# CogitoNTNU/geoguessr-ai

Hardware: AMD Instinct MI355X
Metric: images/sec TinyViT-21M-224 train, 4-heading batch (higher is better)
Workload: dtype fp32 (bf16x3 split MFMA); 1 GPU; tiny_vit_21m_224 4x224x224 panoramas, fwd+bwd+AdamW, soft-CE over 12647 geocells, freeze_all_but_last_stage, DropPath, train-mode BN; panoramas_per_gpu=256, images_per_gpu=1024, global_batch_panoramas=256, parallelism=dp1, precision=fp32_split

## Files before the change

geoguessr-ai_amd/csrc/gemm_split3.hip:

```cpp
#include "common.h"
#include <type_traits>
#include <algorithm>
#include <stdlib.h>
#include <string.h>
#include "../../include/gg.h"
#include "../../include/gg_wgrad_resident.h"
#include "../../include/gg_conv_dgrad_parity.h"

namespace {

struct Split3Params {
    const bf16* A; int64_t lda, plane_a;
    const float* Af; int64_t ldaf;
    const bf16* B; int64_t ldb, plane_b;
    float* C; int64_t ldc;
    const float* bias;
    int M, N, K, tilesM, tilesN;
    int act; float* preact;
    const float* rowscale; int rows_per_scale;
    const float* residual; int64_t ldr;
    const float* dact_preact; int dact;
    bf16* c_planes; int64_t ldp;
    const float* a_stat; const float* a_gamma; const float* a_beta; int a_act;
    float* colstats;
// ... 901 lines not shown
#pragma unroll
        for (int it = 0; it < 4; ++it) r[it] = load1(it, 1);
#pragma unroll
        for (int i = 0; i < 6; ++i) {
            bf16x4 p1, p2, p3;
            split2(t0[i], 0, p1, p2, p3); split2(t0[i], 2, p1, p2, p3);
            store3(i < 4 ? i : i + 3, Yim, p1, p2, p3);
        }
    }
    union Fr { s3_s4 h[2]; bf16x8 v; };
    Fr yf[3][3], xf[2][3];
    auto rd_y = [&](const bf16* ycur, int pl, int t) {
#pragma unroll
        for (int half = 0; half < 2; ++half)
            yf[pl][t].h[half] = __builtin_amdgcn_ds_read_tr16_b64_v4i16((__attribute__((address_space(3))) s3_s4*)(ycur + pl * PY + yoff[t] + half * 512));
    };
    auto rd_x = [&](int ring, int j) {
#pragma unroll
        for (int pl = 0; pl < 3; ++pl)
#pragma unroll
            for (int half = 0; half < 2; ++half)
                xf[ring][pl].h[half] = __builtin_amdgcn_ds_read_tr16_b64_v4i16((__attribute__((address_space(3))) s3_s4*)(Xim + pl * PX + xoff[j] + half * 512));
    };
    auto phase = [&](auto j0_, auto nj_, auto it0_, auto nit_, int s, bf16* ynxt) {
        constexpr int J0 = decltype(j0_)::value, NJ = decltype(nj_)::value, IT0 = decltype(it0_)::value, NIT = decltype(nit_)::value;
        constexpr int Q = 6 * NJ, S = 3 * NIT;
        constexpr int PA[6] = {0, 1, 2, 0, 1, 0}, PB[6] = {2, 1, 0, 1, 0, 0};
        bf16x4 p1, p2, p3;
#pragma unroll
        for (int jj = 0; jj < NJ; ++jj) {
            if (jj + 1 < NJ) rd_x((jj + 1) & 1, J0 + jj + 1);
#pragma unroll
            for (int g = 0; g < 6; ++g) {
#pragma unroll
                for (int nt = 0; nt < 3; ++nt)
                    acc[nt][J0 + jj] = __builtin_amdgcn_mfma_f32_16x16x32_bf16(xf[jj & 1][PA[g]].v, yf[PB[g]][nt].v, acc[nt][J0 + jj], 0, 0, 0);
                const int qi = jj * 6 + g;
                if ((qi * S) % Q < S) {
                    const int ms = (qi * S) / Q, it = IT0 + ms / 3, part = ms % 3;
                    if (part < 2) split2(r[it], 2 * part, p1, p2, p3);
                    else {
                        store3(it, ynxt, p1, p2, p3);
                        r[it] = load1(it, it >= 4 && it < 7 ? s + 1 : s + 2);
                    }
                }
                __builtin_amdgcn_sched_barrier(0);
            }
        }
    };
    for (int s = 0; s < nk; ++s) {
        const bf16* const ycur = Yim + (s & 1) * 3 * PY;
        bf16* const ynxt = Yim + ((s + 1) & 1) * 3 * PY;
        asm volatile("s_waitcnt lgkmcnt(0)" ::: "memory");
        __builtin_amdgcn_s_barrier();
        rd_x(0, 0);
#pragma unroll
        for (int t = 0; t < 3; ++t) rd_y(ycur, 2, t);
#pragma unroll
        for (int t = 0; t < 3; ++t) rd_y(ycur, 1, t);
#pragma unroll
        for (int t = 0; t < 3; ++t) rd_y(ycur, 0, t);
        phase(std::integral_constant<int, 0>{}, std::integral_constant<int, 4>{}, std::integral_constant<int, 4>{}, std::integral_constant<int, 5>{}, s, ynxt);
        asm volatile("s_waitcnt lgkmcnt(0)" ::: "memory");
        __builtin_amdgcn_s_barrier();
        rd_x(0, 4);
        phase(std::integral_constant<int, 4>{}, std::integral_constant<int, 3>{}, std::integral_constant<int, 0>{}, std::integral_constant<int, 4>{}, s, ynxt);
    }
    wait_vm<0>();
    float* out = p.part + (int64_t)slab * p.N * p.K;
#pragma unroll
    for (int nt = 0; nt < 3; ++nt) {
        const int n = 48 * wn + 16 * nt + lr;
#pragma unroll
        for (int j = 0; j < 7; ++j) {
            const int k = 16 * (wk + 4 * j) + 4 * lg;
            if (n < p.N && k < p.K) *reinterpret_cast<f32x4*>(out + (int64_t)n * p.K + k) = acc[nt][j];
        }
    }
}

struct PeDgradParams {
    const float* dy; const bf16* Bp; const float* y; const float* stat; const float* gamma; const float* beta; int act;
    float* dz; float* part;
    int H, W, Cout, tiles_per_img, total_tiles, tiles_per_block;
};
constexpr int PED_N = 48, PED_BM = 128;
__device__ __host__ __forceinline__ int ped_taps_before(int cls) { return cls == 0 ? 0 : cls == 1 ? 1 : cls == 2 ? 3 : 5; }
__global__ __launch_bounds__(256) void pe_dgrad_pack_kernel(const float* __restrict__ Wt, int64_t ldw, int Cout, bf16* __restrict__ out) {
    const int c4n = Cout / 4, total = PED_N * 9 * c4n;
    for (int i = blockIdx.x * blockDim.x + threadIdx.x; i < total; i += gridDim.x * blockDim.x) {
        const int co = (i % c4n) * 4, u = (i / c4n) % 9, c = i / (9 * c4n);
        const int cls = u < 1 ? 0 : u < 3 ? 1 : u < 5 ? 2 : 3, t = u - ped_taps_before(cls);
        const int py = cls >> 1, px = cls & 1, nx = 1 + px, ty = t / nx, tx = t % nx;
        const int ky = py ? (ty ? 0 : 2) : 1, kx = px ? (tx ? 0 : 2) : 1;
        const int Kc = Cout * (1 + py) * (1 + px);
        const f32x4 v = *reinterpret_cast<const f32x4*>(Wt + (int64_t)((ky * 3 + kx) * PED_N + c) * ldw + co);
        bf16x4 p1, p2, p3;
#pragma unroll
        for (int j = 0; j < 4; ++j) {
            bf16 s1_, s2_, s3_;
            gg_split3_rne(v[j], s1_, s2_, s3_);
            p1[j] = s1_; p2[j] = s2_; p3[j] = s3_;
        }
        bf16* q = out + (int64_t)3 * PED_N * Cout * ped_taps_before(cls) + (int64_t)c * Kc + t * Cout + co;
        *reinterpret_cast<bf16x4*>(q) = p1; *reinterpret_cast<bf16x4*>(q + PED_N * Kc) = p2; *reinterpret_cast<bf16x4*>(q + 2 * PED_N * Kc) = p3;
    }
}
__global__ __launch_bounds__(256) void pe_dgrad_split3_kernel(PeDgradParams p) {
    constexpr int BM = PED_BM, BN = PED_N, TM = 2, TN = 3, LDT = BN + 4;
    constexpr int TA = BM * S3_SK, TB = BN * S3_SK;
    constexpr int CPR = BN / 4, RPP = 256 / CPR, NR = (BM + RPP - 1) / RPP;
    extern __shared__ __attribute__((aligned(16))) bf16 s3mem[];
    bf16* const Abuf = s3mem;
    bf16* const Bbuf = s3mem + 3 * TA;
    float* const Ct = reinterpret_cast<float*>(s3mem);
    const int lane = threadIdx.x & 63, wave = __builtin_amdgcn_readfirstlane(threadIdx.x >> 6);
    const int lr = lane & 15, lg = lane >> 4;
    const int H0 = p.H >> 1, W0 = p.W >> 1, npc = H0 * W0, spt = p.Cout >> 5;
    const int dchunk = (lane & 3) ^ s3_swz(lane >> 4);
    const int kq = threadIdx.x & 7, arow = threadIdx.x >> 3;
    int ldsA[4];
#pragma unroll
    for (int j = 0; j < 4; ++j) {
        const int row = arow + 32 * j;
        ldsA[j] = row * S3_SK + (((kq >> 1) ^ s3_swz((row >> 2) & 3)) << 3) + ((kq & 1) << 2);
    }
    const int fslot = (lg ^ s3_swz((lr >> 2) & 3)) * 8;
    const int a_off = (wave * 32 + lr) * S3_SK + fslot, b_off = lr * S3_SK + fslot;
    const int chunk = threadIdx.x % CPR, r0 = threadIdx.x / CPR, c0 = chunk * 4;
    const bool elive = r0 < RPP;
    const f32x4 mu = *reinterpret_cast<const f32x4*>(p.stat + c0), rstd = *reinterpret_cast<const f32x4*>(p.stat + BN + c0);
    const f32x4 ga = *reinterpret_cast<const f32x4*>(p.gamma + c0), be = *reinterpret_cast<const f32x4*>(p.beta + c0);
    f32x4 ssum = {0.f, 0.f, 0.f, 0.f}, qsum = ssum;
    auto split2 = [&](const f32x4& v, int e0, bf16x4& p1, bf16x4& p2, bf16x4& p3) {
#pragma unroll
        for (int e = e0; e < e0 + 2; ++e) {
            bf16 s1_, s2_, s3_;
            gg_split3_rne(v[e], s1_, s2_, s3_);
            p1[e] = s1_; p2[e] = s2_; p3[e] = s3_;
        }
    };
    const int lid = gg_xcd_remap(blockIdx.x, gridDim.x);
    const int t_begin = lid * p.tiles_per_block, t_end = min(t_begin + p.tiles_per_block, p.total_tiles);
    for (int tile = t_begin; tile < t_end; ++tile) {
        const int img = tile / (4 * p.tiles_per_img), rem = tile - img * 4 * p.tiles_per_img;
        const int tin = rem >> 2, cls = rem & 3, py = cls >> 1, px = cls & 1, nx = 1 + px;
        const int Kc = p.Cout * (1 + py) * nx, nk = spt * (1 + py) * nx;
        const int q0 = tin * BM;
        const __amdgpu_buffer_rsrc_t rsA = __builtin_amdgcn_make_buffer_rsrc((void*)(p.dy + (int64_t)img * npc * p.Cout), 0, (int)((unsigned)npc * (unsigned)p.Cout * 4u), 0x00020000);
        unsigned voffA[4];
        bool yin[4], xin[4];
#pragma unroll
        for (int j = 0; j < 4; ++j) {
            const int q = q0 + arow + 32 * j, m = q / W0, n = q - m * W0;
            voffA[j] = q < npc ? (unsigned)q * (unsigned)p.Cout * 4u + kq * 16u : 0xFFFFFFF0u;
            yin[j] = m + 1 < H0; xin[j] = n + 1 < W0;
        }
        __amdgpu_buffer_rsrc_t rsB[3];
#pragma unroll
        for (int i = 0; i < 3; ++i)
            rsB[i] = __builtin_amdgcn_make_buffer_rsrc((void*)(p.Bp + (int64_t)3 * BN * p.Cout * ped_taps_before(cls) + (int64_t)i * BN * Kc), 0, (int)((unsigned)BN * (unsigned)Kc * 2u), 0x00020000);
        const unsigned voffB = (unsigned)(wave * 16 + (lane >> 2)) * (unsigned)Kc * 2u + dchunk * 16u;
        auto issue_b = [&](int st) {
            if (wave < BN / 16 && st < nk) {
                bf16* const base = Bbuf + (st & 1) * 3 * TB;
#pragma unroll
                for (int i = 0; i < 3; ++i)
                    __builtin_amdgcn_raw_ptr_buffer_load_lds(rsB[i], (__attribute__((address_space(3))) void*)(base + i * TB + wave * 512), 16, (int)voffB, st * S3_SK * 2, 0, 0);
            }
        };
        auto load_a1 = [&](int st, int j) -> f32x4 {
            const int t = st / spt, kk = (st - t * spt) * S3_SK, ty = t / nx, tx = t - ty * nx;
            const bool dyv = py && ty, dxv = px && tx;
            const int soff = (((int)dyv * W0 + (int)dxv) * p.Cout + kk) * 4;
            const bool ok = st < nk && (!dyv || yin[j]) && (!dxv || xin[j]);
            return __builtin_bit_cast(f32x4, __builtin_amdgcn_raw_buffer_load_b128(rsA, (int)(ok ? voffA[j] : 0xFFFFFFF0u), soff, 0));
        };
        auto load_a = [&](int st, f32x4 (&r)[4]) {
#pragma unroll
            for (int j = 0; j < 4; ++j) r[j] = load_a1(st, j);
        };
        f32x4 acc[TN][TM], accs[TN][TM];
#pragma unroll
        for (int i = 0; i < TN; ++i)
#pragma unroll
            for (int j = 0; j < TM; ++j) acc[i][j] = accs[i][j] = (f32x4){0.f, 0.f, 0.f, 0.f};
        f32x4 ra[2][4];
        issue_b(0);
        load_a(0, ra[0]);
        load_a(1, ra[1]);
        wait_vm<4>();
        {
            bf16x4 p1, p2, p3;
#pragma unroll
            for (int j = 0; j < 4; ++j) {
                split2(ra[0][j], 0, p1, p2, p3); split2(ra[0][j], 2, p1, p2, p3);
                *reinterpret_cast<bf16x4*>(Abuf + ldsA[j]) = p1; *reinterpret_cast<bf16x4*>(Abuf + TA + ldsA[j]) = p2; *reinterpret_cast<bf16x4*>(Abuf + 2 * TA + ldsA[j]) = p3;
            }
        }
        load_a(2, ra[0]);
        auto stage = [&](int s, f32x4 (&rnext)[4]) {
            const bf16* const curB = Bbuf + (s & 1) * 3 * TB;
            wait_vm<4>();
            asm volatile("s_waitcnt lgkmcnt(0)" ::: "memory");
            __builtin_amdgcn_s_barrier();
            issue_b(s + 1);
            bf16x8 xf[3][TM], wf[3][TN];
#pragma unroll
            for (int pl = 0; pl < 3; ++pl)
#pragma unroll
                for (int mt = 0; mt < TM; ++mt) xf[pl][mt] = *reinterpret_cast<const bf16x8*>(Abuf + pl * TA + a_off + mt * 16 * S3_SK);
            auto rd_b1 = [&](int pl, int nt) { wf[pl][nt] = *reinterpret_cast<const bf16x8*>(curB + pl * TB + b_off + nt * 16 * S3_SK); };
#pragma unroll
            for (int t = 0; t < TN; ++t) rd_b1(2, t);
            asm volatile("s_waitcnt lgkmcnt(0)" ::: "memory");
            __builtin_amdgcn_s_barrier();
            bf16x4 p1, p2, p3;
            constexpr int PA[6] = {0, 1, 2, 0, 1, 0}, PB[6] = {2, 1, 0, 1, 0, 0};
#pragma unroll
            for (int g = 0; g < 6; ++g) {
#pragma unroll
                for (int nt = 0; nt < TN; ++nt) {
#pragma unroll
                    for (int mt = 0; mt < TM; ++mt) {
                        if (g < 5) accs[nt][mt] = __builtin_amdgcn_mfma_f32_16x16x32_bf16(wf[PB[g]][nt], xf[PA[g]][mt], accs[nt][mt], 0, 0, 0);
                        else acc[nt][mt] = __builtin_amdgcn_mfma_f32_16x16x32_bf16(wf[PB[g]][nt], xf[PA[g]][mt], acc[nt][mt], 0, 0, 0);
                    }
                    constexpr int Q = 6 * TN;
                    const int qi = g * TN + nt;
                    if (g < 2 && 2 * nt < TN) { rd_b1(1 - g, 2 * nt); if (2 * nt + 1 < TN) rd_b1(1 - g, 2 * nt + 1); }
                    if ((qi * 12) % Q < 12) {
                        const int ms = (qi * 12) / Q, jj = ms / 3, part = ms % 3;
                        if (part < 2) split2(rnext[jj], 2 * part, p1, p2, p3);
                        else {
                            *reinterpret_cast<bf16x4*>(Abuf + ldsA[jj]) = p1;
                            *reinterpret_cast<bf16x4*>(Abuf + TA + ldsA[jj]) = p2;
                            *reinterpret_cast<bf16x4*>(Abuf + 2 * TA + ldsA[jj]) = p3;
                            rnext[jj] = load_a1(s + 3, jj);
                        }
                    }
                    __builtin_amdgcn_sched_barrier(0);
                }
            }
        };
        for (int s = 0; s < nk; s += 2) {
            stage(s, ra[1]);
            if (s + 1 < nk) stage(s + 1, ra[0]);
        }
        wait_vm<0>();
        f32x4 yv[NR];
        int64_t pix[NR];
#pragma unroll
        for (int i = 0; i < NR; ++i) {
            const int rr = r0 + i * RPP, q = q0 + rr;
            const bool on = elive && rr < BM && q < npc;
            const int m = on ? q / W0 : 0, n = on ? q - m * W0 : 0;
            pix[i] = on ? ((int64_t)img * p.H + 2 * m + py) * p.W + 2 * n + px : -1;
            yv[i] = on ? *reinterpret_cast<const f32x4*>(p.y + pix[i] * BN + c0) : (f32x4){0.f, 0.f, 0.f, 0.f};
        }
        asm volatile("s_waitcnt lgkmcnt(0)" ::: "memory");
        __builtin_amdgcn_s_barrier();
#pragma unroll
        for (int nt = 0; nt < TN; ++nt)
#pragma unroll
            for (int mt = 0; mt < TM; ++mt)
                *reinterpret_cast<f32x4*>(Ct + (wave * 32 + mt * 16 + lr) * LDT + nt * 16 + lg * 4) = acc[nt][mt] + accs[nt][mt];
        __syncthreads();
#pragma unroll
        for (int i = 0; i < NR; ++i) {
            if (pix[i] < 0) continue;
            const f32x4 a = *reinterpret_cast<const f32x4*>(Ct + (r0 + i * RPP) * LDT + c0);
            const f32x4 xh = (yv[i] - mu) * rstd;
            f32x4 o;
#pragma unroll
            for (int j = 0; j < 4; ++j) o[j] = a[j] * gg_act_grad_f32(fmaf(ga[j], xh[j], be[j]), p.act);
            ssum += o;
            qsum += o * xh;
            __builtin_nontemporal_store(o, reinterpret_cast<f32x4*>(p.dz + pix[i] * BN + c0));
        }
        __syncthreads();
    }
    if (elive) {
        *reinterpret_cast<f32x4*>(Ct + (r0 * 2 + 0) * BN + c0) = ssum;
        *reinterpret_cast<f32x4*>(Ct + (r0 * 2 + 1) * BN + c0) = qsum;
    }
    __syncthreads();
    if (threadIdx.x < 2 * BN) {
        float t = 0.f;
        for (int k = 0; k < RPP; ++k) t += Ct[k * 2 * BN + threadIdx.x];
        p.part[(int64_t)blockIdx.x * 2 * BN + threadIdx.x] = t;
    }
}

__global__ __launch_bounds__(256) void split3_kernel(const float* __restrict__ x, int64_t rows, int cols, int64_t ldx, bf16* __restrict__ out) {
    const int64_t n4 = rows * (cols / 4);
    const int64_t plane = rows * cols;
    for (int64_t i = blockIdx.x * (int64_t)blockDim.x + threadIdx.x; i < n4; i += (int64_t)gridDim.x * blockDim.x) {
        const int64_t r = i / (cols / 4);
        const int c = (int)(i - r * (cols / 4)) * 4;
        const f32x4 v = *reinterpret_cast<const f32x4*>(x + r * ldx + c);
        bf16x4 p1, p2, p3;
#pragma unroll
        for (int j = 0; j < 4; ++j) {
            bf16 s1_, s2_, s3_;
            gg_split3_rne(v[j], s1_, s2_, s3_);
            p1[j] = s1_; p2[j] = s2_; p3[j] = s3_;
        }
        *reinterpret_cast<bf16x4*>(out + r * cols + c) = p1;
        *reinterpret_cast<bf16x4*>(out + plane + r * cols + c) = p2;
        *reinterpret_cast<bf16x4*>(out + 2 * plane + r * cols + c) = p3;
    }
}

}

extern "C" int gg_split3_bf16(const float* x, int64_t rows, int cols, int64_t ldx, void* planes, void* stream) {
    GG_CHECK(x && planes && rows > 0 && cols > 0 && (cols & 3) == 0 && (ldx & 3) == 0 && ldx >= cols && ((uintptr_t)x & 15) == 0 && ((uintptr_t)planes & 7) == 0,
             "gg_split3_bf16: bad args (cols %% 4, ldx %% 4, 16-byte aligned x)");
    GG_PROF(GG_CAT_MOVE, 0, 10.0 * rows * cols, stream);
    const int64_t n4 = rows * (cols / 4);
    hipLaunchKernelGGL(split3_kernel, dim3((unsigned)std::min<int64_t>(gg_cdiv(n4, 256), 16384)), dim3(256), 0, (hipStream_t)stream, x, rows, cols, ldx, (bf16*)planes);
    GG_LAUNCH_CHECK();
    return 0;
}

static GgSplit3Route split3_planes_route(int M, int N) {
    const bool big = M > 128;
    GgSplit3Route r;
    r.kernel = big ? GG_SPLIT3_ROUTE_PLANES_256 : GG_SPLIT3_ROUTE_PLANES_128;
    r.tile_n = S3_BN; r.epilogue = 0; r.mapped = 0;
    r.tilesM = (int)gg_cdiv(M, big ? 256 : 128); r.tilesN = (int)gg_cdiv(N, S3_BN);
    r.lds_bytes = big ? (int64_t)2 * 3 * (256 + 128) * S3_SK * sizeof(bf16) : (int64_t)3 * S3_STAGE * sizeof(bf16);
    return r;
}
static int split3_launch(Split3Params& p, void* stream) {
    const int M = p.M, N = p.N, K = p.K;
    const GgSplit3Route r = split3_planes_route(M, N);
    void (*kern)(Split3Params) = r.kernel == GG_SPLIT3_ROUTE_PLANES_256 ? gemm_nt_split3_kernel<256, 128, 4, 2, 2> : gemm_nt_split3_kernel<128, 128, 2, 4, 3>;
    p.tilesM = r.tilesM; p.tilesN = r.tilesN;
    const size_t lds = (size_t)r.lds_bytes;
    GG_TRY(gg_allow_lds_160k(reinterpret_cast<const void*>(kern)));
    const double mn = (double)M * N;
    GG_PROF(GG_CAT_GEMM | GG_CAT_SPLIT_FLAG, 2.0 * M * (double)N * K,
            6.0 * ((double)M * K + (double)N * K) + 4.0 * mn * ((p.C != nullptr) + (p.preact != nullptr) + (p.residual != nullptr) + (p.dact_preact != nullptr)) +
                (p.c_planes ? 6.0 * mn : 0.0), stream);
    hipLaunchKernelGGL(kern, dim3((unsigned)(p.tilesM * p.tilesN)), dim3(512), lds, (hipStream_t)stream, p);
    GG_LAUNCH_CHECK();
    return 0;
}

static int split3_planes_check(const GgSplit3Args* a) {
    GG_CHECK(a && a->a_planes && a->b_planes && (a->C || a->c_planes) && a->M > 0 && a->N > 0 && a->K > 0, "gg_gemm_nt_split3: null pointer / bad shape");
    GG_CHECK((a->K & 7) == 0 && (a->lda & 7) == 0 && (a->ldb & 7) == 0 && a->lda >= a->K && a->ldb >= a->K, "gg_gemm_nt_split3: K, lda, ldb must be multiples of 8, ld >= K");
    GG_CHECK(((uintptr_t)a->a_planes & 15) == 0 && ((uintptr_t)a->b_planes & 15) == 0 && ((uintptr_t)a->C & 15) == 0 && ((uintptr_t)a->c_planes & 7) == 0,
             "gg_gemm_nt_split3: alignment");
    GG_CHECK((int64_t)256 * a->lda * 2 < ((int64_t)1 << 31) && (int64_t)256 * a->ldb * 2 < ((int64_t)1 << 31), "gg_gemm_nt_split3: row pitch too large");
    GG_CHECK((!a->C || a->ldc >= a->N) && (!a->c_planes || a->ldp >= a->N) && (!a->residual || a->ldr >= a->N), "gg_gemm_nt_split3: leading dimension too small");
    GG_CHECK((!a->preact && !a->dact_preact) || a->ldc >= a->N, "gg_gemm_nt_split3: preact / dact_preact use ldc");
    GG_CHECK(!a->rowscale || a->rows_per_scale > 0, "gg_gemm_nt_split3: rowscale needs rows_per_scale");
    GG_CHECK(!(a->dact_preact && a->act), "gg_gemm_nt_split3: act and dact_preact are exclusive");
    GG_CHECK(!a->groups_dev && !a->a_map && !a->c_map, "gg_gemm_nt_split3: row compaction is a form of gg_gemm_nt_split3_af32 only");
    return 0;
}
extern "C" int gg_gemm_nt_split3_ex(const GgSplit3Args* a, void* stream) {
    GG_TRY(split3_planes_check(a));
    Split3Params p;
    p.a_stat = p.a_gamma = p.a_beta = nullptr; p.a_act = 0;
    p.A = (const bf16*)a->a_planes; p.lda = a->lda; p.plane_a = (int64_t)a->M * a->lda; p.Af = nullptr; p.ldaf = 0;
    p.B = (const bf16*)a->b_planes; p.ldb = a->ldb; p.plane_b = (int64_t)a->N * a->ldb;
    p.C = a->C; p.ldc = a->ldc ? a->ldc : a->N; p.bias = a->bias; p.M = a->M; p.N = a->N; p.K = a->K;
    p.act = a->act; p.preact = a->preact; p.rowscale = a->rowscale; p.rows_per_scale = a->rows_per_scale; p.residual = a->residual; p.ldr = a->ldr;
    p.dact_preact = a->dact_preact; p.dact = a->dact; p.c_planes = (bf16*)a->c_planes; p.ldp = a->ldp; p.colstats = nullptr;
// ... 143 lines not shown
    GG_TRY(split3_af32_check(a, (const float*)a->a_planes, a->lda, with_colstats != 0, pro != 0));
    return split3_af32_route(a, with_colstats != 0, pro != 0, *out);
}

extern "C" int gg_gemm_tn_f32_splits(int M, int N, int K);
extern "C" int gg_gemm_tn_split3_splits(int M, int N, int K) {
    const int64_t tiles = gg_cdiv(N, 256) * gg_cdiv(K, 128);
    const int64_t cap = std::max<int64_t>(1, ((int64_t)128 << 20) / ((int64_t)N * K * 4));
    const int64_t smax = std::max<int64_t>(1, std::min<int64_t>(cap, gg_cdiv(M, 1024)));
    int64_t s = 1;
    double best = 0.0;
    for (int64_t c = 1; c <= smax && c * tiles <= 4 * 256; ++c) {
        const double eff = (double)(c * tiles) / (256.0 * (double)gg_cdiv(c * tiles, 256));
        if (eff > best + 0.02) { best = eff; s = c; }
    }
    s = std::min<int64_t>(cap, std::max<int64_t>(s, (5 * (int64_t)gg_gemm_tn_f32_splits(M, N, K) + 3) / 4));
    const int64_t rows = gg_cdiv(gg_cdiv(M, s), 32) * 32;
    return (int)gg_cdiv(M, rows);
}
extern "C" int gg_gemm_tn_split3(const float* dY, int64_t ldy, const float* X, int64_t ldx, int M, int N, int K, const float* rowscale, int rows_per_scale, float* partials,
                                 int splits, void* stream) {
    GG_CHECK(dY && X && partials && M > 0 && N > 0 && K > 0 && splits > 0, "gg_gemm_tn_split3: bad args");
    GG_CHECK((N & 3) == 0 && (K & 3) == 0 && (ldy & 3) == 0 && (ldx & 3) == 0 && ldy >= N && ldx >= K, "gg_gemm_tn_split3: N, K, ldy, ldx must be multiples of 4, ld >= columns");
    GG_CHECK(((uintptr_t)dY & 15) == 0 && ((uintptr_t)X & 15) == 0 && ((uintptr_t)partials & 15) == 0, "gg_gemm_tn_split3: operands and partials must be 16-byte aligned");
    GG_CHECK(!rowscale || rows_per_scale > 0, "gg_gemm_tn_split3: rows_per_scale");
    Split3TnParams p;
    p.dY = dY; p.ldy = ldy; p.X = X; p.ldx = ldx; p.M = M; p.N = N; p.K = K; p.rowscale = rowscale; p.rps = rows_per_scale > 0 ? rows_per_scale : 1; p.part = partials;
    p.last_scale = (M - 1) / p.rps;
    p.rows_per_split = (int)(gg_cdiv(gg_cdiv(M, splits), 32) * 32);
    GG_CHECK((int64_t)p.rows_per_split * (splits - 1) < M, "gg_gemm_tn_split3: more splits than 32-row stages");
    GG_CHECK((int64_t)p.rows_per_split * std::max(ldy, ldx) * 4 < ((int64_t)1 << 31), "gg_gemm_tn_split3: a slab exceeds the 2 GiB descriptor range");
    p.tilesN = (int)gg_cdiv(N, 256); p.tilesK = (int)gg_cdiv(K, 128);
    GG_TRY(gg_allow_lds_160k(reinterpret_cast<const void*>(gemm_tn_split3_kernel)));
    GG_PROF(GG_CAT_GEMM | GG_CAT_SPLIT_FLAG, 2.0 * M * (double)N * K, 4.0 * ((double)M * N + (double)M * K) + 8.0 * splits * (double)N * K, stream);
    hipLaunchKernelGGL(gemm_tn_split3_kernel, dim3((unsigned)(p.tilesN * p.tilesK * splits)), dim3(512), (size_t)2 * 3 * (256 / 32 + 128 / 32) * 1024 * sizeof(bf16), (hipStream_t)stream, p);
    GG_LAUNCH_CHECK();
    return 0;
}

extern "C" int gg_gemm_tn_split3_resident_fits(int N, int K) { return N > 0 && K > 0 && N <= S3R_N && K <= S3R_K; }
extern "C" int gg_gemm_tn_split3_resident_splits(int M, int N, int K) {
    GG_CHECK(M > 0 && N > 0 && K > 0, "gg_gemm_tn_split3_resident_splits: bad shape");
    GG_CHECK(gg_gemm_tn_split3_resident_fits(N, K), "gg_gemm_tn_split3_resident: the %d x %d output does not fit one workgroup (at most %d x %d)", N, K, S3R_N, S3R_K);
    const int64_t cap = std::max<int64_t>(1, ((int64_t)128 << 20) / ((int64_t)N * K * 4));
    int64_t s = std::max<int64_t>(1, std::min<int64_t>(256, M / 256));
    s = std::max<int64_t>(s, (5 * (int64_t)gg_gemm_tn_f32_splits(M, N, K) + 3) / 4);
    s = std::min<int64_t>(std::min<int64_t>(s, cap), gg_cdiv(M, 32));
    const int64_t rows = gg_cdiv(gg_cdiv(M, s), 32) * 32;
    return (int)gg_cdiv(M, rows);
}
extern "C" int gg_gemm_tn_split3_resident(const float* dY, int64_t ldy, const float* X, int64_t ldx, int M, int N, int K, float* partials, int splits, void* stream) {
    GG_CHECK(dY && X && partials && M > 0 && N > 0 && K > 0 && splits > 0, "gg_gemm_tn_split3_resident: bad args");
    GG_CHECK(gg_gemm_tn_split3_resident_fits(N, K), "gg_gemm_tn_split3_resident: the %d x %d output does not fit one workgroup (at most %d x %d)", N, K, S3R_N, S3R_K);
    GG_CHECK((N & 3) == 0 && (K & 3) == 0 && (ldy & 3) == 0 && (ldx & 3) == 0 && ldy >= N && ldx >= K, "gg_gemm_tn_split3_resident: N, K, ldy, ldx must be multiples of 4, ld >= columns");
    GG_CHECK(((uintptr_t)dY & 15) == 0 && ((uintptr_t)X & 15) == 0 && ((uintptr_t)partials & 15) == 0, "gg_gemm_tn_split3_resident: operands and partials must be 16-byte aligned");
    Split3TnResParams p;
    p.dY = dY; p.ldy = ldy; p.X = X; p.ldx = ldx; p.M = M; p.N = N; p.K = K; p.part = partials;
    p.rows_per_split = (int)(gg_cdiv(gg_cdiv(M, splits), 32) * 32);
    GG_CHECK((int64_t)p.rows_per_split * (splits - 1) < M, "gg_gemm_tn_split3_resident: more splits than 32-row stages");
    GG_CHECK(((int64_t)p.rows_per_split + 96) * std::max(ldy, ldx) * 4 < ((int64_t)1 << 31), "gg_gemm_tn_split3_resident: a slab exceeds the 2 GiB descriptor range");
    GG_TRY(gg_allow_lds_160k(reinterpret_cast<const void*>(gemm_tn_split3_resident_kernel)));
    GG_PROF(GG_CAT_GEMM | GG_CAT_SPLIT_FLAG, 2.0 * M * (double)N * K, 4.0 * ((double)M * N + (double)M * K) + 8.0 * splits * (double)N * K, stream);
    hipLaunchKernelGGL(gemm_tn_split3_resident_kernel, dim3((unsigned)splits), dim3(512), (size_t)3 * (S3R_K / 32 + 2 * (S3R_N / 32)) * 1024 * sizeof(bf16), (hipStream_t)stream, p);
    GG_LAUNCH_CHECK();
    return 0;
}

extern "C" int gg_conv3x3s2_dgrad_fits(int H, int W, int Cin, int Cout) {
    return H > 0 && W > 0 && (H & 1) == 0 && (W & 1) == 0 && Cin == PED_N && Cout >= 32 && (Cout & 31) == 0 && (int64_t)(H / 2) * (W / 2) * Cout * 4 < ((int64_t)1 << 31);
}
extern "C" int64_t gg_conv3x3s2_dgrad_planes_bytes(int Cin, int Cout) { return (int64_t)3 * 9 * Cin * Cout * (int64_t)sizeof(bf16); }
extern "C" int gg_conv3x3s2_dgrad_bnbwd_split3(const float* dy, const float* Wt, int64_t ldw, const float* y, const float* stat, const float* gamma, const float* beta, int act,
                                               float* dz, float* part, int nparts, void* planes, int B, int H, int W, int Cin, int Cout, void* stream) {
    GG_CHECK(dy && Wt && y && stat && gamma && beta && dz && part && planes && nparts > 0 && nparts <= 65535 && B > 0, "gg_conv3x3s2_dgrad_bnbwd_split3: bad args");
    GG_CHECK(gg_conv3x3s2_dgrad_fits(H, W, Cin, Cout), "gg_conv3x3s2_dgrad_bnbwd_split3: needs an even input map, Cin = %d and Cout a multiple of 32 (got %d x %d, Cin %d, Cout %d)",
             PED_N, H, W, Cin, Cout);
    GG_CHECK(ldw >= Cout && (ldw & 3) == 0, "gg_conv3x3s2_dgrad_bnbwd_split3: ldw must be a multiple of 4, >= Cout");
    GG_CHECK(((uintptr_t)dy & 15) == 0 && ((uintptr_t)Wt & 15) == 0 && ((uintptr_t)y & 15) == 0 && ((uintptr_t)dz & 15) == 0 && ((uintptr_t)stat & 15) == 0 &&
             ((uintptr_t)gamma & 15) == 0 && ((uintptr_t)beta & 15) == 0 && ((uintptr_t)planes & 15) == 0, "gg_conv3x3s2_dgrad_bnbwd_split3: operands must be 16-byte aligned");
    PeDgradParams p;
    p.dy = dy; p.Bp = (const bf16*)planes; p.y = y; p.stat = stat; p.gamma = gamma; p.beta = beta; p.act = act; p.dz = dz; p.part = part;
    p.H = H; p.W = W; p.Cout = Cout;
    const int64_t npc = (int64_t)(H / 2) * (W / 2);
    p.tiles_per_img = (int)gg_cdiv(npc, PED_BM);
    const int64_t total = (int64_t)B * 4 * p.tiles_per_img;
    GG_CHECK(total < ((int64_t)1 << 31), "gg_conv3x3s2_dgrad_bnbwd_split3: too many tiles");
    p.total_tiles = (int)total;
    p.tiles_per_block = (int)gg_cdiv(total, nparts);
    const double M0 = (double)B * npc;
    {
        GG_PROF(GG_CAT_MOVE, 0, 4.0 * 9 * Cin * Cout + 6.0 * 9 * Cin * Cout, stream);
        hipLaunchKernelGGL(pe_dgrad_pack_kernel, dim3((unsigned)gg_cdiv((int64_t)PED_N * 9 * (Cout / 4), 256)), dim3(256), 0, (hipStream_t)stream, Wt, ldw, Cout, (bf16*)planes);
        GG_LAUNCH_CHECK();
    }
    GG_PROF(GG_CAT_GEMM | GG_CAT_SPLIT_FLAG, 2.0 * M0 * 9.0 * Cin * Cout, 4.0 * M0 * Cout + 6.0 * 9 * Cin * Cout + 2.0 * 4.0 * 4.0 * M0 * Cin + 8.0 * nparts * Cin, stream);
    hipLaunchKernelGGL(pe_dgrad_split3_kernel, dim3((unsigned)nparts), dim3(256), (size_t)(3 * PED_BM + 6 * PED_N) * S3_SK * sizeof(bf16), (hipStream_t)stream, p);
    GG_LAUNCH_CHECK();
    return 0;
}
```

Before: 5815 images/s.

## Stage a split dy spatial tile in LDS once and reuse it across all nine taps

Result: no change. 5835 images/s (median of 6 runs) (+0.3%).

```diff
diff --git a/geoguessr-ai_amd/csrc/gemm_split3.hip b/geoguessr-ai_amd/csrc/gemm_split3.hip
--- a/geoguessr-ai_amd/csrc/gemm_split3.hip
+++ b/geoguessr-ai_amd/csrc/gemm_split3.hip
@@ -1007,18 +1007,21 @@
 struct PeDgradParams {
     const float* dy; const bf16* Bp; const float* y; const float* stat; const float* gamma; const float* beta; int act;
     float* dz; float* part;
-    int H, W, Cout, tiles_per_img, total_tiles, tiles_per_block;
+    int H, W, Cout, tiles_x, tiles_per_img, total_tiles, tiles_per_block;
 };
-constexpr int PED_N = 48, PED_BM = 128;
+constexpr int PED_N = 48, PED_TW = 14, PED_FW = 16, PED_TH = 4, PED_RING = 3;
+constexpr int PED_BT = PED_N * S3_SK;
 __device__ __host__ __forceinline__ int ped_taps_before(int cls) { return cls == 0 ? 0 : cls == 1 ? 1 : cls == 2 ? 3 : 5; }
+__host__ __forceinline__ size_t ped_lds_bytes(int th, int ring, int Cout) {
+    return (size_t)4 * PED_N * sizeof(float) + ((size_t)3 * (Cout / 32) * (th + 1) * PED_FW * S3_SK + (size_t)ring * 3 * PED_BT) * sizeof(bf16);
+}
 __global__ __launch_bounds__(256) void pe_dgrad_pack_kernel(const float* __restrict__ Wt, int64_t ldw, int Cout, bf16* __restrict__ out) {
-    const int c4n = Cout / 4, total = PED_N * 9 * c4n;
+    const int c4n = Cout / 4, spt = Cout >> 5, total = PED_N * 9 * c4n;
     for (int i = blockIdx.x * blockDim.x + threadIdx.x; i < total; i += gridDim.x * blockDim.x) {
         const int co = (i % c4n) * 4, u = (i / c4n) % 9, c = i / (9 * c4n);
         const int cls = u < 1 ? 0 : u < 3 ? 1 : u < 5 ? 2 : 3, t = u - ped_taps_before(cls);
         const int py = cls >> 1, px = cls & 1, nx = 1 + px, ty = t / nx, tx = t % nx;
         const int ky = py ? (ty ? 0 : 2) : 1, kx = px ? (tx ? 0 : 2) : 1;
-        const int Kc = Cout * (1 + py) * (1 + px);
         const f32x4 v = *reinterpret_cast<const f32x4*>(Wt + (int64_t)((ky * 3 + kx) * PED_N + c) * ldw + co);
         bf16x4 p1, p2, p3;
 #pragma unroll
@@ -1027,192 +1030,182 @@
             gg_split3_rne(v[j], s1_, s2_, s3_);
             p1[j] = s1_; p2[j] = s2_; p3[j] = s3_;
         }
-        bf16* q = out + (int64_t)3 * PED_N * Cout * ped_taps_before(cls) + (int64_t)c * Kc + t * Cout + co;
-        *reinterpret_cast<bf16x4*>(q) = p1; *reinterpret_cast<bf16x4*>(q + PED_N * Kc) = p2; *reinterpret_cast<bf16x4*>(q + 2 * PED_N * Kc) = p3;
-    }
-}
+        const int ks = co >> 5, kk = co & 31;
+        bf16* q = out + ((int64_t)(u * spt + ks) * 3 * PED_N + c) * S3_SK + ((((kk >> 3) ^ s3_swz((c >> 2) & 3)) << 3) | (kk & 7));
+        *reinterpret_cast<bf16x4*>(q) = p1; *reinterpret_cast<bf16x4*>(q + PED_BT) = p2; *reinterpret_cast<bf16x4*>(q + 2 * PED_BT) = p3;
+    }
+}
+template <int TH, int R>
 __global__ __launch_bounds__(256) void pe_dgrad_split3_kernel(PeDgradParams p) {
-    constexpr int BM = PED_BM, BN = PED_N, TM = 2, TN = 3, LDT = BN + 4;
-    constexpr int TA = BM * S3_SK, TB = BN * S3_SK;
-    constexpr int CPR = BN / 4, RPP = 256 / CPR, NR = (BM + RPP - 1) / RPP;
+    constexpr int BN = PED_N, TW = PED_TW, FW = PED_FW, TM = TH / 4, TN = 3, NPIX = (TH + 1) * FW, SB = 3 * PED_BT;
+    static_assert(TH % 4 == 0 && R >= 3 && R - 1 <= 9, "one or two tile rows per wave; the ring is filled from the first tile's stages");
     extern __shared__ __attribute__((aligned(16))) bf16 s3mem[];
-    bf16* const Abuf = s3mem;
-    bf16* const Bbuf = s3mem + 3 * TA;
-    float* const Ct = reinterpret_cast<float*>(s3mem);
+    float* const bnt = reinterpret_cast<float*>(s3mem);
+    bf16* const Aimg = s3mem + 4 * BN * 2;
     const int lane = threadIdx.x & 63, wave = __builtin_amdgcn_readfirstlane(threadIdx.x >> 6);
     const int lr = lane & 15, lg = lane >> 4;
-    const int H0 = p.H >> 1, W0 = p.W >> 1, npc = H0 * W0, spt = p.Cout >> 5;
-    const int dchunk = (lane & 3) ^ s3_swz(lane >> 4);
-    const int kq = threadIdx.x & 7, arow = threadIdx.x >> 3;
-    int ldsA[4];
-#pragma unroll
-    for (int j = 0; j < 4; ++j) {
-        const int row = arow + 32 * j;
-        ldsA[j] = row * S3_SK + (((kq >> 1) ^ s3_swz((row >> 2) & 3)) << 3) + ((kq & 1) << 2);
-    }
-    const int fslot = (lg ^ s3_swz((lr >> 2) & 3)) * 8;
-    const int a_off = (wave * 32 + lr) * S3_SK + fslot, b_off = lr * S3_SK + fslot;
-    const int chunk = threadIdx.x % CPR, r0 = threadIdx.x / CPR, c0 = chunk * 4;
-    const bool elive = r0 < RPP;
-    const f32x4 mu = *reinterpret_cast<const f32x4*>(p.stat + c0), rstd = *reinterpret_cast<const f32x4*>(p.stat + BN + c0);
-    const f32x4 ga = *reinterpret_cast<const f32x4*>(p.gamma + c0), be = *reinterpret_cast<const f32x4*>(p.beta + c0);
-    f32x4 ssum = {0.f, 0.f, 0.f, 0.f}, qsum = ssum;
-    auto split2 = [&](const f32x4& v, int e0, bf16x4& p1, bf16x4& p2, bf16x4& p3) {
-#pragma unroll
-        for (int e = e0; e < e0 + 2; ++e) {
-            bf16 s1_, s2_, s3_;
-            gg_split3_rne(v[e], s1_, s2_, s3_);
-            p1[e] = s1_; p2[e] = s2_; p3[e] = s3_;
-        }
-    };
+    const int H0 = p.H >> 1, W0 = p.W >> 1, npc = H0 * W0, spt = p.Cout >> 5, nst = 9 * spt;
+    const int PS = spt * NPIX * S3_SK;
+    bf16* const Bring = Aimg + 3 * PS;
+    float* const red = reinterpret_cast<float*>(Aimg);
     const int lid = gg_xcd_remap(blockIdx.x, gridDim.x);
-    const int t_begin = lid * p.tiles_per_block, t_end = min(t_begin + p.tiles_per_block, p.total_tiles);
+    const int t_begin = min(lid * p.tiles_per_block, p.total_tiles), t_end = min(t_begin + p.tiles_per_block, p.total_tiles);
+    const int gtotal = (t_end - t_begin) * nst;
+    if (threadIdx.x < BN) {
+        bnt[threadIdx.x] = p.stat[threadIdx.x]; bnt[BN + threadIdx.x] = p.stat[BN + threadIdx.x];
+        bnt[2 * BN + threadIdx.x] = p.gamma[threadIdx.x]; bnt[3 * BN + threadIdx.x] = p.beta[threadIdx.x];
+    }
+    const __amdgpu_buffer_rsrc_t rsB = __builtin_amdgcn_make_buffer_rsrc((void*)p.Bp, 0, (int)((unsigned)nst * SB * 2u), 0x00020000);
+    const unsigned voffB = (unsigned)(wave * 512 + lane * 8) * 2u;
+    int gi = 0, bsi = 0, sloti = 0;
+    auto issue_b = [&]() {
+        if (wave < BN / 16 && gi < gtotal) {
+            bf16* const base = Bring + sloti * SB;
+#pragma unroll
+            for (int i = 0; i < 3; ++i)
+                __builtin_amdgcn_raw_ptr_buffer_load_lds(rsB, (__attribute__((address_space(3))) void*)(base + i * PED_BT + wave * 512), 16, (int)voffB, (bsi * SB + i * PED_BT) * 2, 0, 0);
+        }
+        ++gi;
+        bsi = bsi + 1 == nst ? 0 : bsi + 1;
+        sloti = sloti + 1 == R ? 0 : sloti + 1;
+    };
+    int aoff[TM][2];
+#pragma unroll
+    for (int mt = 0; mt < TM; ++mt)
+#pragma unroll
+        for (int dx = 0; dx < 2; ++dx) {
+            const int pix = (wave * TM + mt) * FW + min(lr + dx, FW - 1);
+            aoff[mt][dx] = pix * S3_SK + ((lg ^ s3_swz((pix >> 2) & 3)) << 3);
+        }
+    const int b_off = lr * S3_SK + ((lg ^ s3_swz((lr >> 2) & 3)) << 3);
+    const int c4n = p.Cout >> 2, items = NPIX * c4n;
+    f32x4 ssum[TN], qsum[TN];
+#pragma unroll
+    for (int nt = 0; nt < TN; ++nt) ssum[nt] = qsum[nt] = (f32x4){0.f, 0.f, 0.f, 0.f};
+#pragma unroll
+    for (int j = 0; j < R - 1; ++j) issue_b();
+    int g = 0, slot = 0;
     for (int tile = t_begin; tile < t_end; ++tile) {
-        const int img = tile / (4 * p.tiles_per_img), rem = tile - img * 4 * p.tiles_per_img;
-        const int tin = rem >> 2, cls = rem & 3, py = cls >> 1, px = cls & 1, nx = 1 + px;
-        const int Kc = p.Cout * (1 + py) * nx, nk = spt * (1 + py) * nx;
-        const int q0 = tin * BM;
-        const __amdgpu_buffer_rsrc_t rsA = __builtin_amdgcn_make_buffer_rsrc((void*)(p.dy + (int64_t)img * npc * p.Cout), 0, (int)((unsigned)npc * (unsigned)p.Cout * 4u), 0x00020000);
-        unsigned voffA[4];
-        bool yin[4], xin[4];
-#pragma unroll
-        for (int j = 0; j < 4; ++j) {
-            const int q = q0 + arow + 32 * j, m = q / W0, n = q - m * W0;
-            voffA[j] = q < npc ? (unsigned)q * (unsigned)p.Cout * 4u + kq * 16u : 0xFFFFFFF0u;
-            yin[j] = m + 1 < H0; xin[j] = n + 1 < W0;
-        }
-        __amdgpu_buffer_rsrc_t rsB[3];
-#pragma unroll
-        for (int i = 0; i < 3; ++i)
-            rsB[i] = __builtin_amdgcn_make_buffer_rsrc((void*)(p.Bp + (int64_t)3 * BN * p.Cout * ped_taps_before(cls) + (int64_t)i * BN * Kc), 0, (int)((unsigned)BN * (unsigned)Kc * 2u), 0x00020000);
-        const unsigned voffB = (unsigned)(wave * 16 + (lane >> 2)) * (unsigned)Kc * 2u + dchunk * 16u;
-        auto issue_b = [&](int st) {
-            if (wave < BN / 16 && st < nk) {
-                bf16* const base = Bbuf + (st & 1) * 3 * TB;
-#pragma unroll
-                for (int i = 0; i < 3; ++i)
-                    __builtin_amdgcn_raw_ptr_buffer_load_lds(rsB[i], (__attribute__((address_space(3))) void*)(base + i * TB + wave * 512), 16, (int)voffB, st * S3_SK * 2, 0, 0);
+        const int img = tile / p.tiles_per_img, rem = tile - img * p.tiles_per_img, tyi = rem / p.tiles_x, txi = rem - tyi * p.tiles_x;
+        const int m0 = tyi * TH, n0 = txi * TW;
+        __syncthreads();
+        const float* const dyi = p.dy + (int64_t)img * npc * p.Cout;
+        for (int i0 = threadIdx.x; i0 < items; i0 += 4 * 256) {
+            f32x4 v[4];
+#pragma unroll
+            for (int k = 0; k < 4; ++k) {
+                const int i = i0 + k * 256, pix = i / c4n, c4 = i - pix * c4n, cc = pix & (FW - 1), M = m0 + pix / FW, Nn = n0 + cc;
+                const bool ok = i < items && cc <= TW && M < H0 && Nn < W0;
+                v[k] = ok ? *reinterpret_cast<const f32x4*>(dyi + ((int64_t)M * W0 + Nn) * p.Cout + c4 * 4) : (f32x4){0.f, 0.f, 0.f, 0.f};
             }
-        };
-        auto load_a1 = [&](int st, int j) -> f32x4 {
-            const int t = st / spt, kk = (st - t * spt) * S3_SK, ty = t / nx, tx = t - ty * nx;
-            const bool dyv = py && ty, dxv = px && tx;
-            const int soff = (((int)dyv * W0 + (int)dxv) * p.Cout + kk) * 4;
-            const bool ok = st < nk && (!dyv || yin[j]) && (!dxv || xin[j]);
-            return __builtin_bit_cast(f32x4, __builtin_amdgcn_raw_buffer_load_b128(rsA, (int)(ok ? voffA[j] : 0xFFFFFFF0u), soff, 0));
-        };
-        auto load_a = [&](int st, f32x4 (&r)[4]) {
-#pragma unroll
-            for (int j = 0; j < 4; ++j) r[j] = load_a1(st, j);
-        };
-        f32x4 acc[TN][TM], accs[TN][TM];
+#pragma unroll
+            for (int k = 0; k < 4; ++k) {
+                const int i = i0 + k * 256, pix = i / c4n, co = (i - pix * c4n) * 4, ks = co >> 5, kk = co & 31;
+                if (i >= items) break;
+                bf16x4 p1, p2, p3;
+#pragma unroll
+                for (int e = 0; e < 4; ++e) {
+                    bf16 s1_, s2_, s3_;
+                    gg_split3_rne(v[k][e], s1_, s2_, s3_);
+                    p1[e] = s1_; p2[e] = s2_; p3[e] = s3_;
+                }
+                bf16* const q = Aimg + (ks * NPIX + pix) * S3_SK + ((((kk >> 3) ^ s3_swz((pix >> 2) & 3)) << 3) | (kk & 7));
+                *reinterpret_cast<bf16x4*>(q) = p1; *reinterpret_cast<bf16x4*>(q + PS) = p2; *reinterpret_cast<bf16x4*>(q + 2 * PS) = p3;
+            }
+        }
+        bool live[TM];
+        int64_t pix0[TM];
+#pragma unroll
+        for (int mt = 0; mt < TM; ++mt) {
+            const int Mc = m0 + wave * TM + mt, Nc = n0 + lr;
+            live[mt] = lr < TW && Mc < H0 && Nc < W0;
+            pix0[mt] = (((int64_t)img * p.H + 2 * Mc) * p.W + 2 * Nc) * BN + lg * 4;
+        }
+        f32x4 acc[TN][TM], accs[TN][TM], yv[TN][TM];
 #pragma unroll
         for (int i = 0; i < TN; ++i)
 #pragma unroll
-            for (int j = 0; j < TM; ++j) acc[i][j] = accs[i][j] = (f32x4){0.f, 0.f, 0.f, 0.f};
-        f32x4 ra[2][4];
-        issue_b(0);
-        load_a(0, ra[0]);
-        load_a(1, ra[1]);
-        wait_vm<4>();
-        {
-            bf16x4 p1, p2, p3;
-#pragma unroll
-            for (int j = 0; j < 4; ++j) {
-                split2(ra[0][j], 0, p1, p2, p3); split2(ra[0][j], 2, p1, p2, p3);
-                *reinterpret_cast<bf16x4*>(Abuf + ldsA[j]) = p1; *reinterpret_cast<bf16x4*>(Abuf + TA + ldsA[j]) = p2; *reinterpret_cast<bf16x4*>(Abuf + 2 * TA + ldsA[j]) = p3;
-            }
-        }
-        load_a(2, ra[0]);
-        auto stage = [&](int s, f32x4 (&rnext)[4]) {
-            const bf16* const curB = Bbuf + (s & 1) * 3 * TB;
-            wait_vm<4>();
-            asm volatile("s_waitcnt lgkmcnt(0)" ::: "memory");
-            __builtin_amdgcn_s_barrier();
-            issue_b(s + 1);
-            bf16x8 xf[3][TM], wf[3][TN];
-#pragma unroll
-            for (int pl = 0; pl < 3; ++pl)
-#pragma unroll
-                for (int mt = 0; mt < TM; ++mt) xf[pl][mt] = *reinterpret_cast<const bf16x8*>(Abuf + pl * TA + a_off + mt * 16 * S3_SK);
-            auto rd_b1 = [&](int pl, int nt) { wf[pl][nt] = *reinterpret_cast<const bf16x8*>(curB + pl * TB + b_off + nt * 16 * S3_SK); };
-#pragma unroll
-            for (int t = 0; t < TN; ++t) rd_b1(2, t);
-            asm volatile("s_waitcnt lgkmcnt(0)" ::: "memory");
-            __builtin_amdgcn_s_barrier();
-            bf16x4 p1, p2, p3;
-            constexpr int PA[6] = {0, 1, 2, 0, 1, 0}, PB[6] = {2, 1, 0, 1, 0, 0};
-#pragma unroll
-            for (int g = 0; g < 6; ++g) {
-#pragma unroll
-                for (int nt = 0; nt < TN; ++nt) {
-#pragma unroll
-                    for (int mt = 0; mt < TM; ++mt) {
-                        if (g < 5) accs[nt][mt] = __builtin_amdgcn_mfma_f32_16x16x32_bf16(wf[PB[g]][nt], xf[PA[g]][mt], accs[nt][mt], 0, 0, 0);
-                        else acc[nt][mt] = __builtin_amdgcn_mfma_f32_16x16x32_bf16(wf[PB[g]][nt], xf[PA[g]][mt], acc[nt][mt], 0, 0, 0);
-                    }
-                    constexpr int Q = 6 * TN;
-                    const int qi = g * TN + nt;
-                    if (g < 2 && 2 * nt < TN) { rd_b1(1 - g, 2 * nt); if (2 * nt + 1 < TN) rd_b1(1 - g, 2 * nt + 1); }
-                    if ((qi * 12) % Q < 12) {
-                        const int ms = (qi * 12) / Q, jj = ms / 3, part = ms % 3;
-                        if (part < 2) split2(rnext[jj], 2 * part, p1, p2, p3);
-                        else {
-                            *reinterpret_cast<bf16x4*>(Abuf + ldsA[jj]) = p1;
-                            *reinterpret_cast<bf16x4*>(Abuf + TA + ldsA[jj]) = p2;
-                            *reinterpret_cast<bf16x4*>(Abuf + 2 * TA + ldsA[jj]) = p3;
-                            rnext[jj] = load_a1(s + 3, jj);
+            for (int j = 0; j < TM; ++j) acc[i][j] = accs[i][j] = yv[i][j] = (f32x4){0.f, 0.f, 0.f, 0.f};
+        for (int u = 0; u < 9; ++u) {
+            const int cls = u < 1 ? 0 : u < 3 ? 1 : u < 5 ? 2 : 3, t = u - ped_taps_before(cls), py = cls >> 1, px = cls & 1;
+            const int dyv = py & (px ? t >> 1 : t), dxv = px & t;
+            const bool last_tap = u == 0 || u == 2 || u == 4 || u == 8;
+            const int64_t poff = ((int64_t)py * p.W + px) * BN;
+            for (int ks = 0; ks < spt; ++ks) {
+                if (g + R - 2 < gtotal) wait_vm<3 * (R - 2)>(); else wait_vm<0>();
+                asm volatile("s_waitcnt lgkmcnt(0)" ::: "memory");
+                __builtin_amdgcn_s_barrier();
+                asm volatile("" ::: "memory");
+                issue_b();
+                if (last_tap && ks == spt - 1) {
+#pragma unroll
+                    for (int mt = 0; mt < TM; ++mt)
+                        if (live[mt]) {
+#pragma unroll
+                            for (int nt = 0; nt < TN; ++nt) yv[nt][mt] = *reinterpret_cast<const f32x4*>(p.y + pix0[mt] + poff + nt * 16);
+                        }
+                }
+                const bf16* const curB = Bring + slot * SB;
+                const bf16* const curA = Aimg + (ks * NPIX + dyv * FW) * S3_SK;
+                bf16x8 xf[3][TM], wf[3][TN];
+#pragma unroll
+                for (int pl = 0; pl < 3; ++pl) {
+#pragma unroll
+                    for (int mt = 0; mt < TM; ++mt) xf[pl][mt] = *reinterpret_cast<const bf16x8*>(curA + pl * PS + (dxv ? aoff[mt][1] : aoff[mt][0]));
+                }
+#pragma unroll
+                for (int pl = 2; pl >= 0; --pl) {
+#pragma unroll
+                    for (int nt = 0; nt < TN; ++nt) wf[pl][nt] = *reinterpret_cast<const bf16x8*>(curB + pl * PED_BT + b_off + nt * 16 * S3_SK);
+                }
+                constexpr int PA[6] = {0, 1, 2, 0, 1, 0}, PB[6] = {2, 1, 0, 1, 0, 0};
+#pragma unroll
+                for (int q = 0; q < 6; ++q) {
+#pragma unroll
+                    for (int nt = 0; nt < TN; ++nt) {
+#pragma unroll
+                        for (int mt = 0; mt < TM; ++mt) {
+                            if (q < 5) accs[nt][mt] = __builtin_amdgcn_mfma_f32_16x16x32_bf16(wf[PB[q]][nt], xf[PA[q]][mt], accs[nt][mt], 0, 0, 0);
+                            else acc[nt][mt] = __builtin_amdgcn_mfma_f32_16x16x32_bf16(wf[PB[q]][nt], xf[PA[q]][mt], acc[nt][mt], 0, 0, 0);
                         }
                     }
-                    __builtin_amdgcn_sched_barrier(0);
+                }
+                ++g;
+                slot = slot + 1 == R ? 0 : slot + 1;
+            }
+            if (!last_tap) continue;
+#pragma unroll
+            for (int mt = 0; mt < TM; ++mt) {
+#pragma unroll
+                for (int nt = 0; nt < TN; ++nt) {
+                    if (live[mt]) {
+                        const int c0 = nt * 16 + lg * 4;
+                        const f32x4 mu = *reinterpret_cast<const f32x4*>(bnt + c0), rstd = *reinterpret_cast<const f32x4*>(bnt + BN + c0);
+                        const f32x4 ga = *reinterpret_cast<const f32x4*>(bnt + 2 * BN + c0), be = *reinterpret_cast<const f32x4*>(bnt + 3 * BN + c0);
+                        const f32x4 a = acc[nt][mt] + accs[nt][mt];
+                        const f32x4 xh = (yv[nt][mt] - mu) * rstd;
+                        f32x4 o;
+#pragma unroll
+                        for (int j = 0; j < 4; ++j) o[j] = a[j] * gg_act_grad_f32(fmaf(ga[j], xh[j], be[j]), p.act);
+                        ssum[nt] += o;
+                        qsum[nt] += o * xh;
+                        __builtin_nontemporal_store(o, reinterpret_cast<f32x4*>(p.dz + pix0[mt] + poff + nt * 16));
+                    }
+                    acc[nt][mt] = accs[nt][mt] = (f32x4){0.f, 0.f, 0.f, 0.f};
                 }
             }
-        };
-        for (int s = 0; s < nk; s += 2) {
-            stage(s, ra[1]);
-            if (s + 1 < nk) stage(s + 1, ra[0]);
-        }
-        wait_vm<0>();
-        f32x4 yv[NR];
-        int64_t pix[NR];
-#pragma unroll
-        for (int i = 0; i < NR; ++i) {
-            const int rr = r0 + i * RPP, q = q0 + rr;
-            const bool on = elive && rr < BM && q < npc;
-            const int m = on ? q / W0 : 0, n = on ? q - m * W0 : 0;
-            pix[i] = on ? ((int64_t)img * p.H + 2 * m + py) * p.W + 2 * n + px : -1;
-            yv[i] = on ? *reinterpret_cast<const f32x4*>(p.y + pix[i] * BN + c0) : (f32x4){0.f, 0.f, 0.f, 0.f};
-        }
-        asm volatile("s_waitcnt lgkmcnt(0)" ::: "memory");
-        __builtin_amdgcn_s_barrier();
-#pragma unroll
-        for (int nt = 0; nt < TN; ++nt)
-#pragma unroll
-            for (int mt = 0; mt < TM; ++mt)
-                *reinterpret_cast<f32x4*>(Ct + (wave * 32 + mt * 16 + lr) * LDT + nt * 16 + lg * 4) = acc[nt][mt] + accs[nt][mt];
-        __syncthreads();
-#pragma unroll
-        for (int i = 0; i < NR; ++i) {
-            if (pix[i] < 0) continue;
-            const f32x4 a = *reinterpret_cast<const f32x4*>(Ct + (r0 + i * RPP) * LDT + c0);
-            const f32x4 xh = (yv[i] - mu) * rstd;
-            f32x4 o;
-#pragma unroll
-            for (int j = 0; j < 4; ++j) o[j] = a[j] * gg_act_grad_f32(fmaf(ga[j], xh[j], be[j]), p.act);
-            ssum += o;
-            qsum += o * xh;
-            __builtin_nontemporal_store(o, reinterpret_cast<f32x4*>(p.dz + pix[i] * BN + c0));
-        }
-        __syncthreads();
-    }
-    if (elive) {
-        *reinterpret_cast<f32x4*>(Ct + (r0 * 2 + 0) * BN + c0) = ssum;
-        *reinterpret_cast<f32x4*>(Ct + (r0 * 2 + 1) * BN + c0) = qsum;
+        }
+    }
+    __syncthreads();
+#pragma unroll
+    for (int nt = 0; nt < TN; ++nt) {
+        *reinterpret_cast<f32x4*>(red + ((wave * 16 + lr) * 2 + 0) * BN + nt * 16 + lg * 4) = ssum[nt];
+        *reinterpret_cast<f32x4*>(red + ((wave * 16 + lr) * 2 + 1) * BN + nt * 16 + lg * 4) = qsum[nt];
     }
     __syncthreads();
     if (threadIdx.x < 2 * BN) {
         float t = 0.f;
-        for (int k = 0; k < RPP; ++k) t += Ct[k * 2 * BN + threadIdx.x];
+        for (int k = 0; k < 64; ++k) t += red[k * 2 * BN + threadIdx.x];
         p.part[(int64_t)blockIdx.x * 2 * BN + threadIdx.x] = t;
     }
 }
@@ -1522,19 +1515,24 @@
     p.dy = dy; p.Bp = (const bf16*)planes; p.y = y; p.stat = stat; p.gamma = gamma; p.beta = beta; p.act = act; p.dz = dz; p.part = part;
     p.H = H; p.W = W; p.Cout = Cout;
     const int64_t npc = (int64_t)(H / 2) * (W / 2);
-    p.tiles_per_img = (int)gg_cdiv(npc, PED_BM);
-    const int64_t total = (int64_t)B * 4 * p.tiles_per_img;
+    const size_t lds = ped_lds_bytes(PED_TH, PED_RING, Cout);
+    GG_CHECK(lds <= 160 * 1024, "gg_conv3x3s2_dgrad_bnbwd_split3: the dy tile of Cout = %d channels does not fit the LDS", Cout);
+    p.tiles_x = (int)gg_cdiv(W / 2, PED_TW);
+    p.tiles_per_img = (int)gg_cdiv(H / 2, PED_TH) * p.tiles_x;
+    const int64_t total = (int64_t)B * p.tiles_per_img;
     GG_CHECK(total < ((int64_t)1 << 31), "gg_conv3x3s2_dgrad_bnbwd_split3: too many tiles");
     p.total_tiles = (int)total;
     p.tiles_per_block = (int)gg_cdiv(total, nparts);
     const double M0 = (double)B * npc;
+    void (*kern)(PeDgradParams) = pe_dgrad_split3_kernel<PED_TH, PED_RING>;
+    if (lds > 64 * 1024) GG_TRY(gg_allow_lds_160k(reinterpret_cast<const void*>(kern)));
     {
         GG_PROF(GG_CAT_MOVE, 0, 4.0 * 9 * Cin * Cout + 6.0 * 9 * Cin * Cout, stream);
         hipLaunchKernelGGL(pe_dgrad_pack_kernel, dim3((unsigned)gg_cdiv((int64_t)PED_N * 9 * (Cout / 4), 256)), dim3(256), 0, (hipStream_t)stream, Wt, ldw, Cout, (bf16*)planes);
         GG_LAUNCH_CHECK();
     }
     GG_PROF(GG_CAT_GEMM | GG_CAT_SPLIT_FLAG, 2.0 * M0 * 9.0 * Cin * Cout, 4.0 * M0 * Cout + 6.0 * 9 * Cin * Cout + 2.0 * 4.0 * 4.0 * M0 * Cin + 8.0 * nparts * Cin, stream);
-    hipLaunchKernelGGL(pe_dgrad_split3_kernel, dim3((unsigned)nparts), dim3(256), (size_t)(3 * PED_BM + 6 * PED_N) * S3_SK * sizeof(bf16), (hipStream_t)stream, p);
+    hipLaunchKernelGGL(kern, dim3((unsigned)nparts), dim3(256), lds, (hipStream_t)stream, p);
     GG_LAUNCH_CHECK();
     return 0;
 }
```
